# zhizdev/sparsefusion

Hardware: AMD Instinct MI355X
Metric: novel views/sec, distillation steps (2 NGP renders fwd+bwd + VAE enc/dec + 51-eval PLMS + LPIPS), 256^2 / 32x32 latents, 2-view synthetic hydrant (higher is better)
Workload: dtype bf16 MFMA operands / f32 accumulate (UNet); f32 (NGP render)

## Files before the change

include/sparsefusion_hip.h:

```cpp
#ifndef SPARSEFUSION_HIP_H
#define SPARSEFUSION_HIP_H

#include <stdint.h>

#ifdef __cplusplus
extern "C" {
#endif

#define SF_OK 0
#define SF_ERR_INVALID 1
#define SF_ERR_LAUNCH 2

const char* sf_last_error(void);
int sf_abi_version(void);
int sf_operand_is_f16(void);


int sf_grid_encode_forward(const float* inputs, const float* embeddings,
                           const int32_t* offsets, float* outputs,
                           uint32_t B, uint32_t D, uint32_t C, uint32_t L,
                           float S, uint32_t H, float* dy_dx,
                           uint32_t gridtype, int align_corners,
                           const int32_t* h_offsets, void* stream);

// ... 163 lines not shown
  float* param;
  const float* grad;
  float* exp_avg;
  float* exp_avg_sq;
  uint64_t n;
  float step_size;
  float pad_;
} sf_adam_tensor;
typedef struct {
  sf_adam_tensor t[SF_ADAM_MAX_TENSORS];
  uint32_t chunk_start[SF_ADAM_MAX_TENSORS];
  uint32_t n_tensors;
  float beta1, beta2, eps;
  float bias_correction2_sqrt;
  float one_minus_beta1, one_minus_beta2;
} sf_adam_args;
int sf_adam_multi(const sf_adam_args* args, void* stream);

uint32_t sf_loss_partial_rows(void);
int sf_upsample2x_forward(const float* in, float* out, uint32_t planes, uint32_t h, uint32_t w, void* stream);
int sf_upsample2x_backward(const float* grad_out, float* grad_in, uint32_t planes, uint32_t h, uint32_t w, void* stream);
int sf_render_loss_forward(const float* img, const float* sil, const float* target_rgb, const float* target_mask, uint64_t n_img,
                           uint64_t n_sil, float scaling, float* partial, void* stream);
int sf_render_loss_backward(const float* img, const float* sil, const float* target_rgb, const float* target_mask, uint64_t n_img,
                            uint64_t n_sil, float scaling, float c_rgb, float c_sil, float c_opacity, float c_entropy,
                            const float* grad_loss, float* grad_img, float* grad_sil, void* stream);
int sf_fusion_loss_forward(const float* img, const float* pred, const float* view_weight, const float* sil, uint32_t views,
                           uint64_t per_view_img, uint64_t per_view_sil, float* partial, void* stream);
int sf_fusion_loss_backward(const float* img, const float* pred, const float* view_weight, const float* sil, uint32_t views,
                            uint64_t per_view_img, uint64_t per_view_sil, float c_l1, float c_opacity, float c_entropy,
                            const float* grad_loss, float* grad_img, float* grad_sil, void* stream);

int sf_plan_run(const sf_op* ops, uint32_t n_ops, void* stream);
int sf_plan_profile(const sf_op* ops, uint32_t n_ops, void* stream, float* h_ms);

uint64_t sf_conv_packed_elems(uint32_t Cout, uint32_t cin_pad, uint32_t kh, uint32_t kw);
int sf_conv_pack_weights(const float* h_w, uint32_t Cout, uint32_t Cin,
                         uint32_t cin_pad, uint32_t kh, uint32_t kw,
                         uint16_t* h_out);

int sf_plms_update(const float* x, const float* eps, const float* noise,
                   const float* h_coef6, uint64_t n, float* x_prev, float* x0,
                   void* stream);
int sf_plms_combine(const float* e0, const float* e1, const float* e2,
                    const float* e3, const float* h_c4, uint64_t n, float* out,
                    float* keep_e0, void* stream);
int sf_plms_step(const float* e0, const float* e1, const float* e2, const float* e3,
                 const float* h_c4, float* keep_e0, const float* x, const float* noise,
                 const float* h_coef6, uint64_t n, float* x_prev,
                 const float* row_src, float* row_dst, uint64_t row_n, void* stream);

#ifdef __cplusplus
}
#endif
#endif
```

sparsefusion_amd/_lib.py:

```python
import ctypes as C
import os

import torch

_HERE = os.path.dirname(os.path.abspath(__file__))
_DEFAULT_LIB = "libsparsefusion_hip_f16.so" if os.environ.get("SF_OPERAND", "bf16").lower() in ("f16", "fp16", "half") else "libsparsefusion_hip.so"
LIB_PATH = os.environ.get("SF_HIP_LIB") or os.path.join(_HERE, _DEFAULT_LIB)

_lib = None

c_f32p = C.c_void_p
c_i32p = C.c_void_p
u32 = C.c_uint32
u64 = C.c_uint64


class SfNgpField(C.Structure):
    _fields_ = [("embeddings", C.c_void_p), ("h_offsets", C.c_void_p), ("L", u32), ("S", C.c_float),
                ("H", u32), ("gridtype", u32),
                ("w0", C.c_void_p), ("b0", C.c_void_p), ("w1", C.c_void_p), ("b1", C.c_void_p),
                ("w2", C.c_void_p), ("b2", C.c_void_p), ("bound", C.c_float)]


class SfNgpFieldGrad(C.Structure):
# ... 43 lines not shown
    "sf_march_rays": (C.c_int, [u32, u32, c_i32p, c_f32p, c_f32p, c_f32p, C.c_float, C.c_float, u32, u32, u32,
                                C.c_void_p, c_f32p, c_f32p, c_f32p, c_f32p, c_f32p, c_f32p, C.c_void_p]),
    "sf_composite_rays": (C.c_int, [u32, u32, C.c_float, c_i32p, c_f32p, c_f32p, c_f32p, c_f32p, c_f32p, c_f32p,
                                    c_f32p, C.c_void_p]),
    "sf_adam_multi": (C.c_int, [C.POINTER(SfAdamArgs), C.c_void_p]),
    "sf_loss_partial_rows": (u32, []),
    "sf_upsample2x_forward": (C.c_int, [c_f32p, c_f32p, u32, u32, u32, C.c_void_p]),
    "sf_upsample2x_backward": (C.c_int, [c_f32p, c_f32p, u32, u32, u32, C.c_void_p]),
    "sf_render_loss_forward": (C.c_int, [c_f32p, c_f32p, c_f32p, c_f32p, u64, u64, C.c_float, c_f32p, C.c_void_p]),
    "sf_render_loss_backward": (C.c_int, [c_f32p, c_f32p, c_f32p, c_f32p, u64, u64, C.c_float, C.c_float, C.c_float, C.c_float,
                                          C.c_float, c_f32p, c_f32p, c_f32p, C.c_void_p]),
    "sf_fusion_loss_forward": (C.c_int, [c_f32p, c_f32p, c_f32p, c_f32p, u32, u64, u64, c_f32p, C.c_void_p]),
    "sf_fusion_loss_backward": (C.c_int, [c_f32p, c_f32p, c_f32p, c_f32p, u32, u64, u64, C.c_float, C.c_float, C.c_float,
                                          c_f32p, c_f32p, c_f32p, C.c_void_p]),
    "sf_ngp_density": (C.c_int, [C.POINTER(SfNgpField), c_f32p, u32, c_f32p, c_f32p, C.c_void_p]),
    "sf_ngp_density_lattice": (C.c_int, [C.POINTER(SfNgpField), c_f32p, c_f32p, c_f32p, u32, u32, u32, c_f32p, C.c_void_p]),
    "sf_gaussian3d_workspace_bytes": (u64, [u32, u32, u32]),
    "sf_gaussian3d": (C.c_int, [c_f32p, c_f32p, u32, u32, u32, C.c_float, C.c_float, C.c_void_p, C.c_void_p, u64, C.c_void_p]),
    "sf_mc_workspace_bytes": (u64, [u32, u32, u32]),
    "sf_mc_count": (C.c_int, [c_f32p, u32, u32, u32, C.c_float, C.c_void_p, u64, C.c_void_p, C.c_void_p]),
    "sf_mc_emit": (C.c_int, [c_f32p, u32, u32, u32, C.c_float, C.c_void_p, u64, c_f32p, c_i32p, C.c_void_p]),
    "sf_ngp_render_forward": (C.c_int, [C.POINTER(SfNgpField), c_f32p, c_f32p, c_f32p, u32, u32, C.c_float,
                                        c_f32p, c_f32p, c_f32p, u32, C.c_float, c_f32p, c_f32p, c_f32p, c_f32p,
                                        c_f32p, c_f32p, c_f32p, c_f32p, c_f32p, c_f32p, u64, C.c_void_p]),
    "sf_ngp_render_backward": (C.c_int, [C.POINTER(SfNgpField), C.POINTER(SfNgpFieldGrad), c_f32p, c_f32p,
                                         c_f32p, u32, u32, c_f32p, c_f32p, c_f32p, c_f32p, c_f32p,
                                         C.c_float, c_f32p, c_f32p, u32, c_f32p, c_f32p, u64, C.c_void_p]),
    "sf_ngp_render_workspace_bytes": (u64, [u32, u32]),
    "sf_ngp_render_forward_workspace_bytes": (u64, [u32, u32]),
    "sf_ngp_render_cache_bytes": (u64, [u32, u32]),
    "sf_ngp_render_occ_eval": (C.c_int, [C.POINTER(SfNgpField), c_f32p, c_f32p, c_f32p, c_f32p, C.c_void_p, C.c_float, u32, u32, u32,
                                         c_f32p, C.c_float, u32, c_f32p, c_f32p, c_f32p, C.c_void_p]),
    "sf_plan_run": (C.c_int, [C.POINTER(SfOp), u32, C.c_void_p]),
    "sf_plan_profile": (C.c_int, [C.POINTER(SfOp), u32, C.c_void_p, C.c_void_p]),
    "sf_conv_packed_elems": (u64, [u32, u32, u32, u32]),
    "sf_conv_pack_weights": (C.c_int, [C.c_void_p, u32, u32, u32, u32, u32, C.c_void_p]),
    "sf_plms_update": (C.c_int, [c_f32p, c_f32p, c_f32p, C.c_void_p, u64, c_f32p, c_f32p, C.c_void_p]),
    "sf_plms_combine": (C.c_int, [c_f32p, c_f32p, c_f32p, c_f32p, C.c_void_p, u64, c_f32p, c_f32p, C.c_void_p]),
    "sf_plms_step": (C.c_int, [c_f32p, c_f32p, c_f32p, c_f32p, C.c_void_p, c_f32p, c_f32p, c_f32p, C.c_void_p, u64, c_f32p, c_f32p, c_f32p, u64, C.c_void_p]),
}


_handles = {}


def _load(path):
    if path not in _handles:
        if not os.path.exists(path):
            raise RuntimeError(
                f"{path} is missing: build it with `python -m sparsefusion_amd.build` (`--f16` for the IEEE-half operand build; "
                "there is no CPU fallback for the sparsefusion_amd hot path)")
        handle = C.CDLL(path)
        for name, (res, args) in SIGNATURES.items():
            fn = getattr(handle, name)
            fn.restype = res
            fn.argtypes = args
        _handles[path] = handle
    return _handles[path]


def lib(operand=None):
    global _lib
    if operand is None:
        if _lib is None:
            _lib = _load(LIB_PATH)
        return _lib
# ... 30 lines not shown
```

sparsefusion_amd/csrc/unet_ops.hip:

```cpp

#include "sf_common.h"
#include "plan_ops.h"
#include "sf_dev.h"
#include "gemm_rows.h"
#include "conv_halo.h"
#include "conv_halo_small.h"
#include "conv_igemm.h"
#include "attn_ln.h"
#include <math.h>

typedef __attribute__((ext_vector_type(8))) sf_opnd bf16x8;
typedef __attribute__((ext_vector_type(4))) sf_opnd bf16x4;
typedef __attribute__((ext_vector_type(4))) float f32x4;
typedef __attribute__((address_space(1))) float gfloat;

__device__ __forceinline__ void atomic_add_f32(float* p, float v) {
  (void)__builtin_amdgcn_global_atomic_fadd_f32((gfloat*)p, v);
}
__device__ __forceinline__ float silu_f(float v) { return v / (1.0f + __expf(-v)); }
__device__ __forceinline__ float sigmoid_f(float v) { return 1.0f / (1.0f + __expf(-v)); }
__device__ __forceinline__ float gelu_f(float v) { return 0.5f * v * (1.0f + erff(v * 0.70710678118654752f)); }

__device__ __forceinline__ float wave_sum(float v) {
#pragma unroll
  for (int o = 32; o > 0; o >>= 1) v += __shfl_xor(v, o, 64);
  return v;
}
__device__ __forceinline__ float wave_max(float v) {
#pragma unroll
  for (int o = 32; o > 0; o >>= 1) v = fmaxf(v, __shfl_xor(v, o, 64));
  return v;
}



__global__ __launch_bounds__(256) void k_splitk_reduce(const float* __restrict__ ws, const float* __restrict__ bias,
                                                       const float* __restrict__ resid, float* __restrict__ out, int M,
                                                       int Cout, int npad, int groups, int ldc, int co_off, int accum,
                                                       int relu, int nchw_hw) {
  const long total = (long)M * Cout;
// ... 371 lines not shown
  for (int i = threadIdx.x; i < N; i += 256) out[(long)blockIdx.x * N + i] = (sf_opnd)(expf(x[i] * scale - mx) * inv);
}

__global__ __launch_bounds__(256) void k_unpack_out(const float* __restrict__ in, float* __restrict__ out, int B, int HW,
                                                    int C, int ldi) {
  const long n = (long)B * C * HW;
  for (long i = blockIdx.x * 256L + threadIdx.x; i < n; i += (long)gridDim.x * 256) {
    const int p = (int)(i % HW);
    const long bc = i / HW;
    const int c = (int)(bc % C), b = (int)(bc / C);
    out[i] = in[((long)b * HW + p) * ldi + c];
  }
}
__global__ __launch_bounds__(256) void k_add(const float* __restrict__ a, float* __restrict__ out, long n) {
  for (long i = blockIdx.x * 256L + threadIdx.x; i < n; i += (long)gridDim.x * 256) out[i] += a[i];
}

__global__ void k_time_emb(const float* __restrict__ t, const float* __restrict__ w, float* __restrict__ out, int B,
                           int half) {
  const int i = blockIdx.x * blockDim.x + threadIdx.x;
  if (i >= B * half) return;
  const int b = i / half, j = i - b * half;
  const float fr = t[b] * w[j] * 2.0f * 3.14159265358979323846f;
  float* o = out + (long)b * (1 + 2 * half);
  if (j == 0) o[0] = t[b];
  o[1 + j] = sinf(fr);
  o[1 + half + j] = cosf(fr);
}

template <int WM, int WN>
static void launch_conv(const ConvArgs& a, bool a_fp32, int blocks, hipStream_t st) {
  if (a_fp32) k_conv_igemm<WM, WN, true><<<blocks, 256, 0, st>>>(a);
  else k_conv_igemm<WM, WN, false><<<blocks, 256, 0, st>>>(a);
}

static int conv_glds_depth() { return 4; }
template <int BNF, int NST, bool GN>
static int launch_conv_glds(const ConvArgs& a, int nblk, double* part, int cg, hipStream_t st) {
  static unsigned mask = 0;
  const uint32_t lds = conv_glds_lds_bytes(BNF, NST);
  int dev = 0;
  if (hipGetDevice(&dev) != hipSuccess) SF_FAIL(SF_ERR_LAUNCH, "hipGetDevice failed");
  if (dev >= 32 || !(mask & (1u << dev))) {
    if (hipFuncSetAttribute(reinterpret_cast<const void*>(&k_conv_glds<BNF, NST, GN>), hipFuncAttributeMaxDynamicSharedMemorySize, (int)lds) != hipSuccess)
      SF_FAIL(SF_ERR_LAUNCH, "hipFuncSetAttribute(max dynamic LDS) failed");
    if (dev < 32) mask |= 1u << dev;
  }
  k_conv_glds<BNF, NST, GN><<<nblk, 512, lds, st>>>(a, part, cg);
  SF_CHECK_LAUNCH("conv_glds");
  return SF_OK;
}
static bool conv_halo_enabled() { return true; }
template <int BNF, int NST, bool GN>
static int launch_conv_halo(const ConvArgs& a, int nblk, double* part, int cg, hipStream_t st) {
  static unsigned mask = 0;
  const uint32_t lds = conv_halo_lds_bytes(BNF, NST);
  int dev = 0;
  if (hipGetDevice(&dev) != hipSuccess) SF_FAIL(SF_ERR_LAUNCH, "hipGetDevice failed");
  if (dev >= 32 || !(mask & (1u << dev))) {
    if (hipFuncSetAttribute(reinterpret_cast<const void*>(&k_conv3_halo<BNF, NST, GN>), hipFuncAttributeMaxDynamicSharedMemorySize, (int)lds) != hipSuccess)
      SF_FAIL(SF_ERR_LAUNCH, "hipFuncSetAttribute(max dynamic LDS) failed");
    if (dev < 32) mask |= 1u << dev;
  }
  k_conv3_halo<BNF, NST, GN><<<nblk, 512, lds, st>>>(a, part, cg);
  SF_CHECK_LAUNCH("conv3_halo");
  return SF_OK;
// ... 98 lines not shown
    }
    const int glds = (glds_ok && sel != 1 && sel < 6) ? (sel >= 3 ? sel : conv_glds_depth()) : 0;
    const int halo = (sel == 6 || sel == 7) ? sel - 3 : ((sel == 0 && halo_ok && glds && conv_halo_enabled()) ? glds : 0);
    if (op.flags & 128) {
      double* part = (double*)op.p[6];
      const int cg = op.i[15];
      if (!part || (cg != 4 && cg != 8 && cg != 16) || a.Cout % cg || a.co_off || a.ldc != a.Cout || (a.Ho * a.Wo) % 128)
        SF_FAIL(SF_ERR_INVALID, "conv: GroupNorm-partials epilogue needs whole rows, 128 | Ho*Wo, group width 4 / 8 / 16");
      if (halo) return bnf == 8 ? launch_conv_halo_nst<8, true>(a, nblk, part, cg, halo, st) : launch_conv_halo_nst<4, true>(a, nblk, part, cg, halo, st);
      if (glds) return bnf == 8 ? launch_conv_glds_nst<8, true>(a, nblk, part, cg, glds, st) : launch_conv_glds_nst<4, true>(a, nblk, part, cg, glds, st);
      if (bnf == 8) {
        if (f32) k_conv_lds_gn<8, true><<<nblk, 256, 0, st>>>(a, part, cg); else k_conv_lds_gn<8, false><<<nblk, 256, 0, st>>>(a, part, cg);
      } else if (bnf == 4) {
        if (f32) k_conv_lds_gn<4, true><<<nblk, 256, 0, st>>>(a, part, cg); else k_conv_lds_gn<4, false><<<nblk, 256, 0, st>>>(a, part, cg);
      } else {
        SF_FAIL(SF_ERR_INVALID, "conv: unsupported LDS tile %d", bnf);
      }
      SF_CHECK_LAUNCH("conv_lds_gn");
      return SF_OK;
    }
    if (halo) return bnf == 8 ? launch_conv_halo_nst<8, false>(a, nblk, nullptr, 0, halo, st) : launch_conv_halo_nst<4, false>(a, nblk, nullptr, 0, halo, st);
    if (glds) {
      if (int rc = bnf == 8 ? launch_conv_glds_nst<8, false>(a, nblk, nullptr, 0, glds, st) : launch_conv_glds_nst<4, false>(a, nblk, nullptr, 0, glds, st)) return rc;
      return conv_splitk_tail(op, a, M, st);
    }
    if (bnf == 8) {
      if (f32) k_conv_lds<8, true><<<nblk, 256, 0, st>>>(a); else k_conv_lds<8, false><<<nblk, 256, 0, st>>>(a);
    } else if (bnf == 4) {
      if (f32) k_conv_lds<4, true><<<nblk, 256, 0, st>>>(a); else k_conv_lds<4, false><<<nblk, 256, 0, st>>>(a);
    } else {
      SF_FAIL(SF_ERR_INVALID, "conv: unsupported LDS tile %d", bnf);
    }
    SF_CHECK_LAUNCH("conv_lds");
    return conv_splitk_tail(op, a, M, st);
  }
  switch (tile) {
    case 1 * 16 + 1: launch_conv<1, 1>(a, f32, blocks, st); break;
    case 1 * 16 + 2: launch_conv<1, 2>(a, f32, blocks, st); break;
    case 1 * 16 + 4: launch_conv<1, 4>(a, f32, blocks, st); break;
    case 2 * 16 + 1: launch_conv<2, 1>(a, f32, blocks, st); break;
    case 2 * 16 + 2: launch_conv<2, 2>(a, f32, blocks, st); break;
    case 2 * 16 + 4: launch_conv<2, 4>(a, f32, blocks, st); break;
    case 4 * 16 + 1: launch_conv<4, 1>(a, f32, blocks, st); break;
    case 4 * 16 + 2: launch_conv<4, 2>(a, f32, blocks, st); break;
    case 4 * 16 + 4: launch_conv<4, 4>(a, f32, blocks, st); break;
    default: SF_FAIL(SF_ERR_INVALID, "conv: unsupported wave tile %dx%d", WM, WN);
  }
  SF_CHECK_LAUNCH("conv_igemm");
  return conv_splitk_tail(op, a, M, st);
}

static int lazy_from_op(const sf_op& op, int ibase, int M, LazySrc& lz) {
  lz.mode = op.i[ibase]; lz.groups = op.i[ibase + 1]; lz.npad = op.i[ibase + 2]; lz.M = M;
  lz.a = (const float*)op.p[8]; lz.b = (const float*)op.p[9]; lz.r = (const float*)op.p[10];
  if (lz.mode < 0 || lz.mode > 2) SF_FAIL(SF_ERR_INVALID, "lazy source: unknown mode %d", lz.mode);
  if (lz.mode && !lz.a) SF_FAIL(SF_ERR_INVALID, "lazy source: missing operand");
  if (lz.mode == 1 && (lz.groups < 1 || lz.npad % 4)) SF_FAIL(SF_ERR_INVALID, "lazy source: bad split-K geometry");
  if (lz.mode == 2 && !lz.b) SF_FAIL(SF_ERR_INVALID, "lazy source: gate missing");
  return SF_OK;
}

static int run_gn(const sf_op& op, hipStream_t st) {
  const int B = op.i[0], HW = op.i[1], C1 = op.i[2], C2 = op.i[3];
  const int C = C1 + C2, G = op.i[8] > 0 ? op.i[8] : 8;
  if (C % (4 * G) || C1 % 4 || !op.p[7])
    SF_FAIL(SF_ERR_INVALID, "gn_act: unsupported shape HW=%d C=%d G=%d (or missing stats buffer)", HW, C, G);
// ... 408 lines not shown
```

sparsefusion_amd/plan.py:

```python
import torch

from . import _lib

OP_CONV, OP_GN_ACT, OP_LN, OP_GEMV, OP_ATTN, OP_GCA_POOL, OP_ELTWISE, OP_MEMSET, OP_TIME_EMB, OP_SPLITK_REDUCE = range(1, 11)
OP_FCONV, OP_SLOTS, OP_GCA, OP_INITX, OP_GN_FINALIZE = 14, 15, 16, 17, 18
FNORM_NONE, FNORM_GN_SELF, FNORM_GN_SLOTS, FNORM_LN, FNORM_ATTN = range(5)
LDS_MAX = 163840
SKIP_SCALE = 2 ** -0.5


class _Arena:

    def __init__(self, nbytes=None, device=None):
        self.off = 0
        self.buf = torch.empty(nbytes, dtype=torch.uint8, device=device) if nbytes else None

    def alloc(self, nbytes):
        nbytes = (nbytes + 255) // 256 * 256
        off = self.off
        self.off += nbytes
        return (self.buf.data_ptr() + off) if self.buf is not None else (1 << 20) + off


class _T:
    __slots__ = ("ptr", "rows", "C", "HW", "lazy", "slots", "writer", "twin")

    def __init__(self, ptr, rows, C, HW=None):
        self.ptr, self.rows, self.C, self.HW = ptr, rows, C, HW
        self.lazy = None
        self.slots = None
        self.twin = None
        self.writer = None


class PlanOwner:
    conv_waves_target = 1024
    lds_conv_min_blocks = 0
    lds_mid_min_rows = 0
    lds_mid_min_batch = 8
    gn_epilogue = False
    gn_one = True
    ln_wave = True
    tb_stride = 0
    lazy_consumers = 0
    ss_total = 0
    tile_override = None

    def conv_tiling(self, m_frags, n_frags, KS, pixshuf=False):
        ov = self.tile_override
        if ov and (m_frags, n_frags, KS, bool(pixshuf)) in ov:
            return ov[(m_frags, n_frags, KS, bool(pixshuf))]
        best = None
        mfma = m_frags * n_frags * KS
        w_bytes = n_frags * KS * 1024
        for WM in (1, 2, 4):
            if m_frags % WM or (m_frags <= 4 and WM != m_frags and m_frags in (1, 2, 4)):
                continue
            for WN in (1, 2, 4):
                if n_frags % WN:
                    continue
                tiles = (m_frags // WM) * (n_frags // WN)
                for groups in ((1,) if pixshuf else (1, 2, 4, 8, 16, 32)):
                    if groups > 1 and KS // (4 * groups) < 2:
                        continue
                    waves = tiles * groups * 4
                    util = min(1.0, waves / self.conv_waves_target)
                    t_hbm = w_bytes / 4.0e12 / util
                    t_l2 = mfma * 1024 * (1.0 / WN + 1.0 / WM) / 12.0e12 / util
                    t_mfma = mfma * 20 / (1024 * 2.1e9) / util
                    t_part = (2.0 * groups * m_frags * n_frags * 1024 / 3.0e12 + 2.0e-6) if groups > 1 else 0.0
                    cost = max(t_hbm, t_l2, t_mfma) + t_part + 1e-9 * WM * WN
                    if best is None or cost < best[0]:
                        best = (cost, WM, WN, groups)
        return best[1], best[2], best[3]


class Plan:

# ... 97 lines not shown
        lds_min = self.u.lds_conv_min_blocks
        mid = self.u.lds_mid_min_rows if B >= self.u.lds_mid_min_batch else 0
        if lds_min and n_frags >= 4 and (not pixshuf or (mid and M >= mid and Cout % 4 == 0)):
            bnf = 8 if n_frags > 4 else 4
            blocks = ((m_frags + 7) // 8) * ((n_frags + bnf - 1) // bnf)
            if bnf == 8 and blocks < 256:
                bnf, blocks = 4, ((m_frags + 7) // 8) * ((n_frags + 3) // 4)
            halo = (k == 3 and stride == 1 and pad == 1 and not x_f32 and x.C % 64 == 0 and W % 16 == 0 and H % 8 == 0 and M % 128 == 0
                    and Cout % 4 == 0 and ldc % 4 == 0 and co_off % 4 == 0 and (Ho, Wo) == (H, W) and not pixshuf)
            if blocks >= (min(lds_min, 64) if halo else lds_min) and not pixshuf:
                tile, groups = 256 + bnf, 1
                if twin is not None and ldc == Cout and co_off == 0:
                    twin_ws = twin.ptr
            elif mid and M >= mid:
                glds_ok = not x_f32 and x.C % 64 == 0 and Cout % 4 == 0 and ldc % 4 == 0 and co_off % 4 == 0
                stages = KS // 2 if glds_ok else (KS + 1) // 2
                g = 1 if pixshuf else max(1, min(256 // blocks, stages // 4, 16))
                if glds_ok and k == 3 and stride == 1 and pad == 1 and H == W and H in (4, 8) and not pixshuf:
                    g = max(1, min(256 // blocks, x.C // 128, 16))
                tile, groups = 256 + bnf, g
        ws, wi = 0, 0
        if groups > 1:
            wi = self.acquire_ws(groups * M * n_frags * 16 * 4)
            ws = self.ws_ptrs[wi]
        elif twin_ws:
            ws = twin_ws
        defer = bool(defer and not relu and not gelu and 1 < groups <= defer_max_groups and not accum and not pixshuf and co_off == 0 and ldc == Cout == out.C and M == out.rows
                     and (self.u.lazy_consumers & 1))
        bias, res = self.wptr(bname) if bname else 0, resid.ptr if resid else 0
        slots = 0
        if want_slots and pixshuf and tile < 256 and (Cout // 4) % 16 == 0 and ldc % 16 == 0 and co_off % 16 == 0 and (Ho * Wo) % 16 == 0 and not accum:
            slots = self.misc.alloc(4 * M // 16 * (ldc // 16) * 2 * 4)
        nchw = bool(nchw and groups > 1 and not defer and not accum and not resid and tile < 256 and co_off == 0 and ldc == Cout)
        self.op(OP_CONV, (1 if x_f32 else 0) | (2 if pixshuf else 0) | (4 if accum else 0) | (8 if defer else 0) |
                (16 if upsampled else 0) | (32 if relu else 0) | (64 if gelu else 0) | (256 if nchw else 0),
                p=(x.ptr, w_ptr if w_ptr is not None else self.wptr(wname), bias, out.ptr, res, ws, 0, slots),
                i=(B, H, W, x.C, Ho, Wo, Cout, ldc, co_off, k, k, stride, pad, groups, tile))
        if defer:
            out.lazy = ("splitk", ws, bias, res, groups, n_frags * 16, wi)
            self.ws_owners[wi] = out
        out.slots = slots or None
        self.last_conv_nchw = nchw
        out.writer = self.ops[-1] if (tile >= 256 and co_off == 0 and ldc == Cout == out.C and M == out.rows) else None
        out.twin = twin if (twin is not None and tile >= 256 and groups == 1 and ws == twin.ptr) else None
        return Ho, Wo

    def gn_act(self, x, skip, gname, ss_ptr, out, raw=None, silu=True, groups=8, eps=1e-5):
        C1, C2 = x.C, (skip.C if skip else 0)
        self.need(skip)
        lp, li = self.take_lazy(x, ("splitk", "gate"))
        stats = self.zero.alloc(self.B * groups * 2 * 8)
        ready = 0
        wr = x.writer
        cg = (C1 // groups) if not skip else 0
        if (self.u.gn_epilogue and wr is not None and not (wr.flags & 128) and li[0] == 0 and cg in (4, 8, 16)
                and x.HW and x.HW % 128 == 0 and x.rows == self.B * x.HW):
            part = self.misc.alloc(x.rows // 128 * groups * 2 * 8)
            wr.flags |= 128
            wr.p[6] = part or None
            wr.i[15] = cg
            self.op(OP_GN_FINALIZE, 0, p=(part, stats), i=(self.B, x.HW // 128, groups))
            ready = 2
        self.op(OP_GN_ACT, (0 if silu else 1) | ready | (0 if self.u.gn_one else 4),
                p=(x.ptr, skip.ptr if skip else 0, self.wptr(gname + ".weight"), self.wptr(gname + ".bias"), ss_ptr, out.ptr,
                   raw.ptr if raw else 0, stats) + lp,
                i=(self.B, x.HW, C1, C2, self.u.tb_stride) + li + (groups,), f=(eps, SKIP_SCALE))

    def ln(self, x, gname, bname, out, C, rows, eps=1e-5, gelu=False, out_f32=False, resid=None, twin=None):
# ... 33 lines not shown
```

sparsefusion_amd/unet.py:

```python
import math
import os

import numpy as np
import torch
import torch.nn as nn

from . import _lib
from .plan import (FNORM_ATTN, FNORM_GN_SELF, FNORM_GN_SLOTS, FNORM_LN, FNORM_NONE, LDS_MAX, OP_ATTN, OP_CONV, OP_ELTWISE, OP_FCONV, OP_GCA,
                   OP_GCA_POOL, OP_GEMV, OP_GN_ACT, OP_GN_FINALIZE, OP_INITX, OP_LN, OP_MEMSET, OP_SLOTS, OP_SPLITK_REDUCE, OP_TIME_EMB,
                   SKIP_SCALE, Plan, PlanOwner, _T)

PAIR_TILES = {(1, 1, 1), (1, 1, 2), (1, 2, 2), (2, 2, 2), (4, 2, 2)}
PIPE_TILES = {(1, 1, 4), (1, 2, 4), (1, 1, 6), (1, 2, 6), (2, 1, 6), (2, 2, 6), (2, 1, 8), (2, 2, 8), (2, 1, 12), (2, 2, 12), (4, 1, 16), (4, 2, 16)}
CONV3S_VARIANTS = {(5, 256, 5, 2, 2), (5, 256, 3, 2, 2), (4, 256, 4, 1, 1), (4, 256, 2, 1, 1), (4, 512, 4, 1, 2), (4, 512, 2, 1, 2),
                   (3, 512, 3, 1, 1), (3, 1024, 3, 1, 1), (5, 256, 5, 4, 2), (5, 256, 3, 4, 2),
                   (4, 256, 2, 2, 1), (4, 256, 2, 2, 2), (4, 512, 2, 2, 2), (3, 512, 3, 2, 1), (3, 1024, 3, 2, 1), (3, 1024, 3, 2, 2)}
CONV3S_RC_VARIANTS = {(5, 256, 256, 256, 3, 2, 2), (4, 512, 256, 512, 2, 1, 2), (3, 1024, 512, 1024, 3, 1, 1)}
ATTN_LDS_BYTES = 8 * 16 * 36 * 4 + 2 * 8 * 4 * 68 * 4
TILE_PICKS = {(4, 32, 128, False): (1, 2, 8),
              (4, 128, 32, True): (1, 1, 1),
              (16, 64, 16, True): (1, 2, 1),
              (64, 1, 72, False): (1, 1, 4),
              (64, 16, 128, False): (2, 4, 4), (16, 32, 128, False): (1, 4, 4), (4, 64, 256, False): (1, 2, 4),
              (4, 64, 288, False): (1, 4, 4), (4, 256, 32, True): (1, 2, 1), (16, 128, 32, True): (1, 4, 1),
              (64, 64, 16, True): (1, 2, 1)}

SWITCHES = (
    ("conv_waves_target", 1024, "waves wanted per conv launch (4 per CU) before split-K stops"),
    ("lds_conv_min_blocks", 96, "use k_conv_lds when a layer has at least this many 128 x 128 output tiles"),
    ("lds_mid_min_rows", 128, "r06: convs of >= this many rows that have too few 128-row tiles for lds_conv_min_blocks run on the LDS-tiled kernels with split-K groups (Plan.conv); 0 = off"),
    ("merged_down_conv4", True, "r06: the merged 3x3 + 1x1 conv of the last Downsample on k_conv4_gn<64, 0, false> at B = 1; False: k_conv_igemm"),
    ("rc_small_tiles", 32, "r06: bit mask of map sides (32 | 16 | 8) whose B >= 2 (conv1 || res_conv) pairs keep the B = 1 tile of k_conv3s_rc (32: B = 2 eval 1.155 -> 1.139 ms, B = 4 1.562 -> 1.520; 32 | 16: B = 4 1.580, B = 8 2.451 -> 2.550)"),
    ("gn_one", True, "r06: GroupNorm passes of B >= 32 plans (B * 8 >= 256 workgroups) in one launch (k_gn_one); False: k_gn_stats + k_gn_apply everywhere"),
    ("lds_mid_min_batch", 8, "... in plans of at least this many images (the B = 1 .. 4 plans keep their measured kernels)"),
    ("unfused_min_rows_4", 256, "r06: 4x4-level ResnetBlocks with B*16 >= this leave the fused kernels (as unfused_min_rows at 32x32 / 16x16; measured: B = 8 loses 0.12 ms, B = 16 gains 0.22, B = 32 0.49); 0 = never"),
    ("unfused_min_rows_8", 1024, "... 8x8 level (k_conv3_halo_sm; measured: B = 8 loses 0.14 ms, B = 16 gains 0.04, B = 32 0.56)"),
    ("unfused_lin_min_rows", 256, "r06: attention / feed-forward linears of the 4x4 level with >= this many token rows leave the fused kernels (measured: B = 16 3.683 -> 3.670 ms, B = 32 4.664 -> 4.472)"),
    ("unfused_min_rows_16", 4096, "r06: the 16x16 level's own threshold (0 = unfused_min_rows; measured with k_gemm_rows_ks / the r06 plans: B = 16 3.641 -> 3.313 ms; 2048 rows lose: B = 8 2.454 -> 2.512)"),
    ("unfused_min_rows_32", 0, "... 32x32 level (4096 rows lose: B = 4 1.575 -> 1.686 ms)"),
    ("unfused_min_rows", 8192, "ResnetBlocks with B*H*W >= this at the 32x32 / 16x16 levels leave the fused kernels (_Plan.resnet; measured r03: B = 8 eval 3.33 -> 2.96 ms, B = 32 11.5 -> 7.8 ms, B = 4 unchanged)"),
    ("lazy_consumers", 3, "bit 0: split-K reductions, bit 1: gated residuals are materialised by their first consumer"),
    ("fused", True, "GroupNorm inside the conv launches (k_conv_fused) wherever the layer fits; False = the first-round plan"),
    ("pair_res_conv", True, "conv1 || res_conv of a ResnetBlock in one launch"),
    ("res_conv_beside_pool", True, "4x4 gca blocks: the res_conv shares the GlobalContext pooling launch instead"),
    ("initx_direct", True, "latent half of the init conv as one direct-convolution launch"),
    ("big_tile_min_batch", 2, "batch from which the 8x8 / 16x16 / 32x32 maps use 32- / 32- / 64-pixel tiles (r03: B = 2 eval 1.70 -> 1.50 ms, B = 4 2.62 -> 2.02, B = 32 16.4 -> 11.5; at B = 1 they would leave half the CUs idle; 999 = never)"),
    ("gca_epilogue_pool", True, "GlobalContext pooling in conv2's epilogue (False = k_gca_pool launch)"),
    ("fconv_pipe", True, "slot-GroupNorm 3x3 convs on k_conv_fused_pipe (staging || matrix work)"),
    ("producer_slots", True, "r04: k_init_x / the Upsample epilogue leave their consumers' statistics slots, the final conv's split-K reduction writes NCHW (False: the r03 k_slots / k_unpack_out launches; parity tests)"),
    ("attn_in_out_proj", True, "the 16-token attention core in the prologue of its output projection (False: k_attn16 launch; parity tests)"),
    ("ln_wave", True, "r05: LayerNorm of <= 256 rows of 512 | 1024 | 2048 channels on k_layernorm_wave (False: op flag 4 = k_layernorm)"),
    ("gate_t", True, "r05: GlobalContext gate with a compile-time hidden width (k_gca_gate_t; False: k_gca_gate)"),
    ("conv4_reduce_min_batch", 4, "r05: from this batch on a 4x4 split-K conv1 is reduced by its own launch instead of by conv2's gather (0 = never)"),
    ("conv4_mb", True, "r05: even B: the 4x4 GroupNorm-self convs run 2 | 4 images per workgroup (k_conv4_gn_mb; False = op field i[19] bit 0)"),
    ("conv4_slices_max_batch", 4, "r05: up to this batch the 4x4 GroupNorm-self convs keep 4 input-channel slices (= k_conv4_gn's geometry); 0 = the workgroup-count rule alone"),
    ("conv3s", True, "r06: the recurring single-source slot-GroupNorm 3x3 convs on k_conv3s (compile-time geometry, csrc/fused_conv3s.h); False: op field i[19] bit 1 = k_conv_fused_pipe"),
    ("conv3s_tw32", 8, "r06: tile width of k_conv3s's 2-D pixel tiles per map size (0 = full-width strips)"),
    ("conv3s_tw16", 4, "... 16x16 maps"),
    ("conv3s_tw8", 0, "... 8x8 maps"),
    ("conv4", True, "r05: the 4x4 level's GroupNorm-self 3x3 convs on k_conv4_gn (csrc/fused_conv4.h); False: op flag 128 = k_conv_fused (parity tests)"),
    ("use_hip_graph", True, "replay one captured hipGraph per eval instead of ~370 host launches"),
)

# ... 774 lines not shown
        self._locals = dict(dim=dim, dim_mults=tuple(dim_mults), num_resnet_blocks=num_resnet_blocks, layer_attns=layer_attns,
                            layer_cross_attns=layer_cross_attns, cond_images_channels=cond_images_channels, channels=channels,
                            attn_pool_text=attn_pool_text, cond_dim=cond_dim, attn_dim_head=attn_dim_head, attn_heads=attn_heads,
                            ff_mult=ff_mult, learned_sinu_pos_emb_dim=learned_sinu_pos_emb_dim,
                            max_conditional_len=max_conditional_len, image_size=image_size)
        if attn_heads * attn_dim_head != 512 or attn_dim_head != 64:
            raise NotImplementedError("attention kernel is built for 8 heads x 64")
        spec = unet_param_spec(dim, tuple(dim_mults), self.nres, self.attns, cond_images_channels, channels, self.cond_dim,
                               attn_heads, attn_dim_head, ff_mult, learned_sinu_pos_emb_dim, max_conditional_len)
        self.spec_shapes = dict(spec)
        g = torch.Generator().manual_seed(0)
        for name, shape in spec:
            _register(self, name, self._default_init(name, shape, g))
        self.ss_offset, off = {}, 0
        for name, shape in spec:
            if name.endswith(".time_mlp.1.weight"):
                self.ss_offset[name[:-len(".time_mlp.1.weight")]] = off
                off += shape[0]
        self.ss_total = off
        self.tb_off = {}
        for name, shape in spec:
            if name.endswith(".to_context.1.weight"):
                self.tb_off[name[:-len(".to_context.1.weight")]] = off
                off += 2 * shape[0]
            elif name.endswith(".cross_attn.fn.to_kv.weight"):
                self.tb_off[name[:-len(".to_kv.weight")]] = off
                off += 2 * shape[0]
        self.tb_stride = (off + 63) // 64 * 64
        for name, default, _ in SWITCHES:
            setattr(self, name, default)
        self._pack_cache = None
        self._plans = {}
        self.tile_override = dict(TILE_PICKS)

    @staticmethod
    def _default_init(name, shape, g):
        if name.startswith("final_conv"):
            return torch.zeros(shape)
        if name.endswith(".g") or name.endswith("groupnorm.weight") or name in ("norm_cond.weight",) or name.endswith("to_context.0.weight"):
            return torch.ones(shape)
        if name.endswith("bias"):
            return torch.zeros(shape)
        if name.endswith("null_kv") or name.startswith("null_conditional") or name.endswith("weights"):
            return torch.randn(shape, generator=g)
        fan_in = int(np.prod(shape[1:])) if len(shape) > 1 else shape[0]
        return (torch.rand(shape, generator=g) * 2 - 1) / math.sqrt(fan_in)

    def set_switches(self, spec):
        pairs = [kv.split("=") for kv in spec.split(",") if kv]
        unknown = [name for name, _ in pairs if name not in {n for n, _, _ in SWITCHES}]
        if unknown:
            raise KeyError(f"Unet.set_switches: no planner switch named {unknown} (unet.SWITCHES)")
        for name, value in pairs:
            setattr(self, name, int(value))
        self.drop_plans()
        return self

    def cast_model_parameters(self, *, lowres_cond, conditional_embed_dim, channels, channels_out, cond_on_z):
        if lowres_cond or cond_on_z or channels != self.channels or channels_out != self.channels_out:
            raise NotImplementedError("only the first, unconditional-on-text unet of a cascade is supported")
        return self

    def to_config_and_state_dict(self):
        return self._locals, self.state_dict()

    @classmethod
# ... 270 lines not shown
```

Baseline: 17.50.

## Add compile-time-geometry implicit GEMM conv kernel for B=1 eval layers

Adds k_conv_igemm_t, a templated implicit-GEMM convolution whose map size, channels, kernel, stride, tiling and split-K group count are compile-time constants. Seven specific B=1 UNet convs (split-K downsamples and pixel-shuffle 1x1 upsamples with fused SiLU and GroupNorm slot statistics) are routed to it through a new op flag. The point is to remove runtime index arithmetic and let the compiler fully unroll and software-pipeline register prefetch for these unique shapes. In exchange it adds more kernel instantiations, a switch bitmask, and a launch counter. Layers that do not match fall back to the generic kernel.

```diff
diff --git a/include/sparsefusion_hip.h b/include/sparsefusion_hip.h
--- a/include/sparsefusion_hip.h
+++ b/include/sparsefusion_hip.h
@@ -219,6 +219,7 @@
                             const float* grad_loss, float* grad_img, float* grad_sil, void* stream);
 
 int sf_plan_run(const sf_op* ops, uint32_t n_ops, void* stream);
+uint64_t sf_conv_igemm_t_launches(void);
 int sf_plan_profile(const sf_op* ops, uint32_t n_ops, void* stream, float* h_ms);
 
 uint64_t sf_conv_packed_elems(uint32_t Cout, uint32_t cin_pad, uint32_t kh, uint32_t kw);
diff --git a/sparsefusion_amd/_lib.py b/sparsefusion_amd/_lib.py
--- a/sparsefusion_amd/_lib.py
+++ b/sparsefusion_amd/_lib.py
@@ -99,6 +99,7 @@
     "sf_ngp_render_occ_eval": (C.c_int, [C.POINTER(SfNgpField), c_f32p, c_f32p, c_f32p, c_f32p, C.c_void_p, C.c_float, u32, u32, u32,
                                          c_f32p, C.c_float, u32, c_f32p, c_f32p, c_f32p, C.c_void_p]),
     "sf_plan_run": (C.c_int, [C.POINTER(SfOp), u32, C.c_void_p]),
+    "sf_conv_igemm_t_launches": (u64, []),
     "sf_plan_profile": (C.c_int, [C.POINTER(SfOp), u32, C.c_void_p, C.c_void_p]),
     "sf_conv_packed_elems": (u64, [u32, u32, u32, u32]),
     "sf_conv_pack_weights": (C.c_int, [C.c_void_p, u32, u32, u32, u32, u32, C.c_void_p]),
diff --git a/sparsefusion_amd/csrc/conv_igemm_t.h b/sparsefusion_amd/csrc/conv_igemm_t.h
--- /dev/null
+++ b/sparsefusion_amd/csrc/conv_igemm_t.h
@@ -0,0 +1,187 @@
+#pragma once
+#include "sf_dev.h"
+#include "conv_lds.h"
+
+#define SF_IGT_SPLITK 0
+#define SF_IGT_PIXSHUF 1
+
+#define SF_IGEMM_T_VARIANTS(X) \
+  X(5, 256, 256, 4, 2, 1, 0, 2, 2, 4, 1, 0) \
+  X(4, 256, 512, 4, 2, 1, 0, 1, 2, 8, 1, 0) \
+  X(3, 512, 1024, 4, 2, 1, 0, 1, 1, 4, 1, 0) \
+  X(2, 1024, 4096, 1, 1, 0, 0, 1, 1, 1, 1, 1) \
+  X(3, 1024, 2048, 1, 1, 0, 0, 1, 1, 1, 1, 1) \
+  X(4, 512, 1024, 1, 1, 0, 0, 1, 2, 1, 1, 1) \
+  X(5, 256, 4, 3, 1, 1, 0, 1, 1, 4, 1, 0)
+
+constexpr int sf_igt_log2(int v) { return v <= 1 ? 0 : 1 + sf_igt_log2(v >> 1); }
+
+#ifndef SF_IGT_KNOCKOUT
+#define SF_IGT_KNOCKOUT 0
+#endif
+
+template <int HL, int CIN, int COUT, int K, int STRIDE, int PAD, int UPS, int WM, int WN, int GROUPS, bool A_FP32, int EPI>
+SF_KERNEL(256) void k_conv_igemm_t(ConvArgs a) {
+  constexpr int H = 1 << HL, HO = (H + 2 * PAD - K) / STRIDE + 1, HOL = sf_igt_log2(HO), M = HO * HO;
+  constexpr int CCH = CIN / 32, CCL = sf_igt_log2(CCH), KS = K * K * CCH, NF = (COUT + 15) / 16, NPAD = NF * 16;
+  constexpr int MT = M / 16 / WM, NT = NF / WN, SPW = (KS + GROUPS * 4 - 1) / (GROUPS * 4);
+  constexpr bool RAGGED = SPW * GROUPS * 4 != KS;
+  constexpr int STEP_REGS = WM * (A_FP32 ? 8 : 4) + WN * 4;
+  constexpr int D = SPW * STEP_REGS <= 96 ? SPW : (96 / STEP_REGS < 2 ? 2 : 96 / STEP_REGS);
+  constexpr int LDC = COUT / 4;
+  static_assert((1 << HOL) == HO && (1 << CCL) == CCH && CIN % 32 == 0, "k_conv_igemm_t: power-of-two map and channel chunks");
+  static_assert(M % (16 * WM) == 0 && NF % WN == 0, "k_conv_igemm_t: the tiles divide the output evenly (no clamped fragments)");
+  static_assert(EPI == SF_IGT_SPLITK ? GROUPS > 1 : (GROUPS == 1 && COUT % 64 == 0 && M % 16 == 0), "k_conv_igemm_t: epilogue kind");
+  static_assert(H * H * CIN < (1 << 28) && NF * KS * 64 < (1 << 27) && GROUPS * M * NPAD < (1 << 29), "k_conv_igemm_t: 32-bit offsets");
+
+  sf_touch_kernarg<(int)sizeof(ConvArgs)>();
+  SF_SHARED __attribute__((aligned(16))) float red[3][WM * WN * 4 * 64];
+  const int lane = threadIdx.x & 63, wave = sf_uniform((int)(threadIdx.x >> 6));
+  const int tile = blockIdx.x % (MT * NT), grp = blockIdx.x / (MT * NT);
+  const int nt = tile % NT, mt = tile / NT;
+  const int k0 = (grp * 4 + wave) * SPW;
+  const int cgrp = (lane >> 4) * 8;
+
+  float bq[WN];
+#pragma unroll
+  for (int ni = 0; ni < WN; ++ni) bq[ni] = EPI == SF_IGT_PIXSHUF ? a.bias[(nt * WN + ni) * 16 + (lane & 15)] : 0.0f;
+
+  int py[WM], px[WM];
+#pragma unroll
+  for (int mi = 0; mi < WM; ++mi) {
+    const int m = (mt * WM + mi) * 16 + (lane & 15);
+    py[mi] = (m >> HOL) * STRIDE - PAD;
+    px[mi] = (m & (HO - 1)) * STRIDE - PAD;
+  }
+  const float* in32 = reinterpret_cast<const float*>(a.in);
+  const sf_opnd* in16 = reinterpret_cast<const sf_opnd*>(a.in);
+
+  f32x4 ra[D][WM][2];
+  bf16x8 rh[D][WM], rb[D][WN];
+  bool ain[D][WM];
+  auto request = [&](int i, int s) {
+    int ks = k0 + i;
+    if (RAGGED) ks = ks < KS ? ks : KS - 1;
+    const int tap = ks >> CCL, cc = ks & (CCH - 1);
+    const int ky = K == 1 ? 0 : tap / K, kx = K == 1 ? 0 : tap - ky * K;
+#pragma unroll
+    for (int ni = 0; ni < WN; ++ni)
+      rb[s][ni] = SF_IGT_KNOCKOUT == 2 ? sf_zero8() : a.w[((nt * WN + ni) * KS + ks) * 64 + lane];
+#pragma unroll
+    for (int mi = 0; mi < WM; ++mi) {
+      const int iy = py[mi] + ky, ix = px[mi] + kx;
+      ain[s][mi] = PAD == 0 || ((unsigned)iy < (unsigned)H && (unsigned)ix < (unsigned)H);
+      const int off = (ain[s][mi] ? ((iy >> UPS) * (H >> UPS) + (ix >> UPS)) * CIN : 0) + cc * 32 + cgrp;
+      if (SF_IGT_KNOCKOUT == 1) {
+        ra[s][mi][0] = ra[s][mi][1] = f32x4{0.f, 0.f, 0.f, 0.f};
+        rh[s][mi] = sf_zero8();
+      } else if (A_FP32) {
+        ra[s][mi][0] = *reinterpret_cast<const f32x4*>(in32 + off);
+        ra[s][mi][1] = *reinterpret_cast<const f32x4*>(in32 + off + 4);
+      } else {
+        rh[s][mi] = *reinterpret_cast<const bf16x8*>(in16 + off);
+      }
+    }
+  };
+#pragma unroll
+  for (int i = 0; i < D; ++i) request(i, i);
+
+  f32x4 acc[WM][WN];
+#pragma unroll
+  for (int mi = 0; mi < WM; ++mi)
+#pragma unroll
+    for (int ni = 0; ni < WN; ++ni) acc[mi][ni] = f32x4{0.f, 0.f, 0.f, 0.f};
+
+#pragma unroll
+  for (int i = 0; i < SPW; ++i) {
+    const int s = i % D;
+    bf16x8 fa[WM], fb[WN];
+#pragma unroll
+    for (int ni = 0; ni < WN; ++ni) fb[ni] = rb[s][ni];
+#pragma unroll
+    for (int mi = 0; mi < WM; ++mi) {
+      bf16x8 v;
+      if (A_FP32) {
+        const f32x4 lo = ra[s][mi][0], hi = ra[s][mi][1];
+        v[0] = (sf_opnd)lo[0]; v[1] = (sf_opnd)lo[1]; v[2] = (sf_opnd)lo[2]; v[3] = (sf_opnd)lo[3];
+        v[4] = (sf_opnd)hi[0]; v[5] = (sf_opnd)hi[1]; v[6] = (sf_opnd)hi[2]; v[7] = (sf_opnd)hi[3];
+      } else {
+        v = rh[s][mi];
+      }
+      fa[mi] = ain[s][mi] ? v : sf_zero8();
+    }
+    if (i + D < SPW) request(i + D, s);
+    if (!RAGGED || k0 + i < KS) {
+#pragma unroll
+      for (int mi = 0; mi < WM; ++mi)
+#pragma unroll
+        for (int ni = 0; ni < WN; ++ni) acc[mi][ni] = sf_mfma16(fa[mi], fb[ni], acc[mi][ni]);
+    }
+  }
+
+  if (wave > 0) {
+#pragma unroll
+    for (int mi = 0; mi < WM; ++mi)
+#pragma unroll
+      for (int ni = 0; ni < WN; ++ni)
+#pragma unroll
+        for (int r = 0; r < 4; ++r) red[wave - 1][((mi * WN + ni) * 4 + r) * 64 + lane] = acc[mi][ni][r];
+  }
+  sf_sync();
+  if (wave != 0) return;
+#pragma unroll
+  for (int mi = 0; mi < WM; ++mi)
+#pragma unroll
+    for (int ni = 0; ni < WN; ++ni)
+#pragma unroll
+      for (int r = 0; r < 4; ++r) {
+        const int idx = ((mi * WN + ni) * 4 + r) * 64 + lane;
+        acc[mi][ni][r] += red[0][idx] + red[1][idx] + red[2][idx];
+      }
+  if (SF_IGT_KNOCKOUT == 3) {
+#ifndef SF_HOST_EMU
+#pragma unroll
+    for (int mi = 0; mi < WM; ++mi)
+#pragma unroll
+      for (int ni = 0; ni < WN; ++ni) asm volatile("" ::"v"(acc[mi][ni]), "v"(bq[ni]));
+#endif
+    return;
+  }
+
+#pragma unroll
+  for (int mi = 0; mi < WM; ++mi) {
+#pragma unroll
+    for (int ni = 0; ni < WN; ++ni) {
+      const int nf = nt * WN + ni;
+      const int n = nf * 16 + (lane & 15);
+      const int m0 = (mt * WM + mi) * 16 + (lane >> 4) * 4;
+      if (EPI == SF_IGT_SPLITK) {
+#pragma unroll
+        for (int r = 0; r < 4; ++r) a.ws[(grp * M + m0 + r) * NPAD + n] = acc[mi][ni][r];
+      } else {
+        float bv = bq[ni];
+        SF_USE_FROM_HERE(bv);
+        float v[4], sm = 0.0f, sq = 0.0f;
+#pragma unroll
+        for (int r = 0; r < 4; ++r) {
+          v[r] = sf_silu(acc[mi][ni][r] + bv);
+          sm += v[r];
+          sq = fmaf(v[r], v[r], sq);
+        }
+        sm = sf_wave_sum(sm);
+        sq = sf_wave_sum(sq);
+        if (lane == 0) {
+          float* sl = a.slots_out + (((mt * WM + mi) * 4 + (nf & 3)) * (LDC >> 4) + (nf >> 2)) * 2;
+          sl[0] = sm;
+          sl[1] = sq;
+        }
+        const int c = n >> 2, ii = (n >> 1) & 1, jj = n & 1;
+#pragma unroll
+        for (int r = 0; r < 4; ++r) {
+          const int m = m0 + r, oy = m >> HOL, ox = m & (HO - 1);
+          a.out[((2 * oy + ii) * (2 * HO) + 2 * ox + jj) * LDC + c] = v[r];
+        }
+      }
+    }
+  }
+}
diff --git a/sparsefusion_amd/csrc/unet_ops.hip b/sparsefusion_amd/csrc/unet_ops.hip
--- a/sparsefusion_amd/csrc/unet_ops.hip
+++ b/sparsefusion_amd/csrc/unet_ops.hip
@@ -6,6 +6,7 @@
 #include "conv_halo.h"
 #include "conv_halo_small.h"
 #include "conv_igemm.h"
+#include "conv_igemm_t.h"
 #include "attn_ln.h"
 #include <math.h>
 
@@ -443,6 +444,24 @@
 static void launch_conv(const ConvArgs& a, bool a_fp32, int blocks, hipStream_t st) {
   if (a_fp32) k_conv_igemm<WM, WN, true><<<blocks, 256, 0, st>>>(a);
   else k_conv_igemm<WM, WN, false><<<blocks, 256, 0, st>>>(a);
+}
+
+static unsigned long long g_igemm_t_launches = 0;
+extern "C" uint64_t sf_conv_igemm_t_launches(void) { return g_igemm_t_launches; }
+static bool launch_conv_t(const ConvArgs& a, int WM, int WN, bool a_fp32, int blocks, hipStream_t st) {
+  if (a.B != 1 || a.H != a.W || a.kh != a.kw || a.accum || a.resid || a.relu || a.co_off) return false;
+  const int epi = a.pixshuf ? SF_IGT_PIXSHUF : SF_IGT_SPLITK;
+  if (a.pixshuf ? (!a.slots_out || !a.bias || a.ldc * 4 != a.Cout || a.groups != 1) : (a.groups < 2 || !a.ws)) return false;
+#define SF_TRY_IGT(hl_, cin_, cout_, k_, s_, p_, ups_, wm_, wn_, g_, f32_, epi_) \
+  if (a.H == (1 << hl_) && a.Cin == cin_ && a.Cout == cout_ && a.kh == k_ && a.stride == s_ && a.pad == p_ && a.ups == ups_ && WM == wm_ && \
+      WN == wn_ && a.groups == g_ && a_fp32 == (bool)f32_ && epi == epi_ && a.Ho == ((1 << hl_) + 2 * p_ - k_) / s_ + 1 && a.Wo == a.Ho) { \
+    k_conv_igemm_t<hl_, cin_, cout_, k_, s_, p_, ups_, wm_, wn_, g_, (bool)f32_, epi_><<<blocks, 256, 0, st>>>(a); \
+    ++g_igemm_t_launches; \
+    return true; \
+  }
+  SF_IGEMM_T_VARIANTS(SF_TRY_IGT)
+#undef SF_TRY_IGT
+  return false;
 }
 
 static int conv_glds_depth() { return 4; }
@@ -607,6 +626,10 @@
       SF_FAIL(SF_ERR_INVALID, "conv: unsupported LDS tile %d", bnf);
     }
     SF_CHECK_LAUNCH("conv_lds");
+    return conv_splitk_tail(op, a, M, st);
+  }
+  if ((op.flags & 512) && launch_conv_t(a, WM, WN, f32, blocks, st)) {
+    SF_CHECK_LAUNCH("conv_igemm_t");
     return conv_splitk_tail(op, a, M, st);
   }
   switch (tile) {
diff --git a/sparsefusion_amd/plan.py b/sparsefusion_amd/plan.py
--- a/sparsefusion_amd/plan.py
+++ b/sparsefusion_amd/plan.py
@@ -44,6 +44,8 @@
     tb_stride = 0
     lazy_consumers = 0
     ss_total = 0
+    igemm_t = 0
+    igemm_t_variants = ()
     tile_override = None
 
     def conv_tiling(self, m_frags, n_frags, KS, pixshuf=False):
@@ -207,8 +209,13 @@
         if want_slots and pixshuf and tile < 256 and (Cout // 4) % 16 == 0 and ldc % 16 == 0 and co_off % 16 == 0 and (Ho * Wo) % 16 == 0 and not accum:
             slots = self.misc.alloc(4 * M // 16 * (ldc // 16) * 2 * 4)
         nchw = bool(nchw and groups > 1 and not defer and not accum and not resid and tile < 256 and co_off == 0 and ldc == Cout)
+        igt = False
+        if self.u.igemm_t and tile < 256 and B == 1 and H == W and (Ho, Wo) == ((H + 2 * pad - k) // stride + 1,) * 2 and not (accum or res or relu or gelu or co_off):
+            key = (H.bit_length() - 1, x.C, Cout, k, stride, pad, int(bool(upsampled)), WM, WN, groups, int(bool(x_f32)), 1 if pixshuf else 0)
+            if key in self.u.igemm_t_variants and H == 1 << key[0] and (self.u.igemm_t >> self.u.igemm_t_variants.index(key)) & 1:
+                igt = bool(slots and bias and ldc * 4 == Cout) if pixshuf else groups > 1
         self.op(OP_CONV, (1 if x_f32 else 0) | (2 if pixshuf else 0) | (4 if accum else 0) | (8 if defer else 0) |
-                (16 if upsampled else 0) | (32 if relu else 0) | (64 if gelu else 0) | (256 if nchw else 0),
+                (16 if upsampled else 0) | (32 if relu else 0) | (64 if gelu else 0) | (256 if nchw else 0) | (512 if igt else 0),
                 p=(x.ptr, w_ptr if w_ptr is not None else self.wptr(wname), bias, out.ptr, res, ws, 0, slots),
                 i=(B, H, W, x.C, Ho, Wo, Cout, ldc, co_off, k, k, stride, pad, groups, tile))
         if defer:
diff --git a/sparsefusion_amd/unet.py b/sparsefusion_amd/unet.py
--- a/sparsefusion_amd/unet.py
+++ b/sparsefusion_amd/unet.py
@@ -16,6 +16,9 @@
                    (3, 512, 3, 1, 1), (3, 1024, 3, 1, 1), (5, 256, 5, 4, 2), (5, 256, 3, 4, 2),
                    (4, 256, 2, 2, 1), (4, 256, 2, 2, 2), (4, 512, 2, 2, 2), (3, 512, 3, 2, 1), (3, 1024, 3, 2, 1), (3, 1024, 3, 2, 2)}
 CONV3S_RC_VARIANTS = {(5, 256, 256, 256, 3, 2, 2), (4, 512, 256, 512, 2, 1, 2), (3, 1024, 512, 1024, 3, 1, 1)}
+IGEMM_T_VARIANTS = ((5, 256, 256, 4, 2, 1, 0, 2, 2, 4, 1, 0), (4, 256, 512, 4, 2, 1, 0, 1, 2, 8, 1, 0), (3, 512, 1024, 4, 2, 1, 0, 1, 1, 4, 1, 0),
+                    (2, 1024, 4096, 1, 1, 0, 0, 1, 1, 1, 1, 1), (3, 1024, 2048, 1, 1, 0, 0, 1, 1, 1, 1, 1), (4, 512, 1024, 1, 1, 0, 0, 1, 2, 1, 1, 1),
+                    (5, 256, 4, 3, 1, 1, 0, 1, 1, 4, 1, 0))
 ATTN_LDS_BYTES = 8 * 16 * 36 * 4 + 2 * 8 * 4 * 68 * 4
 TILE_PICKS = {(4, 32, 128, False): (1, 2, 8),
               (4, 128, 32, True): (1, 1, 1),
@@ -29,6 +32,7 @@
     ("conv_waves_target", 1024, "waves wanted per conv launch (4 per CU) before split-K stops"),
     ("lds_conv_min_blocks", 96, "use k_conv_lds when a layer has at least this many 128 x 128 output tiles"),
     ("lds_mid_min_rows", 128, "r06: convs of >= this many rows that have too few 128-row tiles for lds_conv_min_blocks run on the LDS-tiled kernels with split-K groups (Plan.conv); 0 = off"),
+    ("igemm_t", 127, "the one-of-a-kind implicit GEMMs of the B = 1 eval on k_conv_igemm_t (compile-time geometry, csrc/conv_igemm_t.h; op flag 512): bit j = row j of IGEMM_T_VARIANTS; 0: k_conv_igemm"),
     ("merged_down_conv4", True, "r06: the merged 3x3 + 1x1 conv of the last Downsample on k_conv4_gn<64, 0, false> at B = 1; False: k_conv_igemm"),
     ("rc_small_tiles", 32, "r06: bit mask of map sides (32 | 16 | 8) whose B >= 2 (conv1 || res_conv) pairs keep the B = 1 tile of k_conv3s_rc (32: B = 2 eval 1.155 -> 1.139 ms, B = 4 1.562 -> 1.520; 32 | 16: B = 4 1.580, B = 8 2.451 -> 2.550)"),
     ("gn_one", True, "r06: GroupNorm passes of B >= 32 plans (B * 8 >= 256 workgroups) in one launch (k_gn_one); False: k_gn_stats + k_gn_apply everywhere"),
@@ -869,6 +873,7 @@
         self._pack_cache = None
         self._plans = {}
         self.tile_override = dict(TILE_PICKS)
+        self.igemm_t_variants = IGEMM_T_VARIANTS
 
     @staticmethod
     def _default_init(name, shape, g):
```

After: 17.77, median of 6. 1.02x the previous value.
